# nghiapq77/face-recognition-cpp-tensorrt

Hardware: AMD Instinct MI355X
Metric: faces/sec end-to-end (detect+embed+match), 640x640 batch=32, 1M gallery (higher is better)
Workload: dtype f16 MFMA recogniser convs (fp32 accumulate) + fp32-accurate detector (fp32 MFMA, fp16 hi/lo-split MFMA for the 64-channel 3x3 convs) + int8-screened coarse scan (fp16 MFMA on exactly widened int8 rows) + exact f32 re-rank match (bit-identical to the exact f32 scan)

## Files before the change

### face-recognition-cpp-tensorrt_amd/csrc/kernels_arc_s2.hip

```cpp
#include "frt_kernels.h"
#include "frt_se_device.h"

#include <type_traits>

namespace {

constexpr int PROW = 144;

__device__ constexpr int kSub[9] = {0, 0, 0, 0, 1, 2, 2, 3, 3};
__device__ constexpr int kDr[9] = {0, 0, 1, 1, 0, 0, 1, 0, 0};
__device__ constexpr int kDc[9] = {0, 1, 0, 1, 0, 0, 0, 0, 1};
__device__ constexpr int kLen[4] = {4, 1, 2, 2};
__device__ constexpr int kRowPar[4] = {1, 0, 1, 0};
__device__ constexpr int kColPar[4] = {1, 0, 0, 1};

template <int NT, int PP, bool SEP = false, bool SCF = false>
__global__ __launch_bounds__(256, 1) void conv_s2_kernel(ConvMfmaArgs p, int R, int n_img, int linear) {
    constexpr int PLANE_B = PP * 4096;
    constexpr int LA = 2, WR = 3, BFD = 2;
    extern __shared__ __attribute__((aligned(16))) char smem[];
    const int tid = threadIdx.x, lane = tid & 63, wave = tid >> 6;
    const int r = lane & 31, hi = lane >> 5;
    const int H = p.H, W = p.W, Ho = p.Ho, Wo = p.Wo, Wq = Wo + 1;
    const int NPp = n_img * (R + 1) * Wq;
    const int strips_per_img = Ho / R;
    const int n_valid = n_img * R * Wo;

    const int n_co_tiles = p.Cout >> 7;
    const int nblk = gridDim.x, bq = nblk >> 3, brem = nblk & 7;
    const int xcd = blockIdx.x & 7, slot = blockIdx.x >> 3;
    const int lid = (xcd < brem ? xcd * (bq + 1) : brem * (bq + 1) + (xcd - brem) * bq) + slot;
    const int co_tile = lid % n_co_tiles, strip = lid / n_co_tiles;
    const int co_base = co_tile * 128, cow = wave * 32;
    const int img0 = (strip / strips_per_img) * n_img;
    const int oy0 = (strip % strips_per_img) * R;
    const int n_chunks = p.Cin >> 6;

    int poff[4][PP];
    const int n_sc = SCF ? (p.Csc >> 6) : 0;
    int poff_sc[SCF ? PP : 1];
    {
        const int plane_px = (R + 1) * Wq;
        const float inv_plane = 1.0f / (float)plane_px, inv_row = 1.0f / (float)Wq;
#pragma unroll
        for (int q = 0; q < PP; ++q) {
            const int g = (q * 4 + wave) * 64 + lane;
            const int px = g / 9, pos = g - px * 9;
            int il = (int)(((float)px + 0.5f) * inv_plane);
            int rem = px - il * plane_px;
            if (rem < 0) { --il; rem += plane_px; } else if (rem >= plane_px) { ++il; rem -= plane_px; }
            int i = (int)(((float)rem + 0.5f) * inv_row);
            int j = rem - i * Wq;
            if (j < 0) { --i; j += Wq; } else if (j >= Wq) { ++i; j -= Wq; }
            const int b = img0 + il;
            const bool live = pos < 8 && px < NPp && b < p.B;
            const int ye = 2 * (oy0 + i), xe = 2 * j;
#pragma unroll
            for (int s = 0; s < 4; ++s) {
                const int y = ye - kRowPar[s], x = xe - kColPar[s];
                poff[s][q] = (live && y >= 0 && y < H && x >= 0 && x < W) ? ((b * H + y) * W + x) * p.Cin + pos * 8 : -1;
            }
            if constexpr (SCF) poff_sc[q] = (live && ye < H && xe < W) ? ((b * H + ye) * W + xe) * p.Csc + pos * 8 : -1;
        }
    }
    const half_t *wfrag = p.wf + ((long)((co_base + cow) >> 5) * n_chunks) * (9 * 4 * 512) + lane * 8;
    int pbase[NT];
#pragma unroll
    for (int j = 0; j < NT; ++j) {
        const int sl = j * 32 + r;
        int pidx = 0;
        if (linear) {
            pidx = sl < R * Wq ? sl : 0;
        } else if (sl < n_valid) {
            const int per = R * Wo;
            int il = (int)(((float)sl + 0.5f) * (1.0f / (float)per));
            int rem = sl - il * per;
            if (rem < 0) { --il; rem += per; } else if (rem >= per) { ++il; rem -= per; }
            int rr = (int)(((float)rem + 0.5f) * (1.0f / (float)Wo));
            int cc = rem - rr * Wo;
            if (cc < 0) { --rr; cc += Wo; } else if (cc >= Wo) { ++rr; cc -= Wo; }
            pidx = (il * (R + 1) + rr) * Wq + cc;
        }
        pbase[j] = pidx * PROW + hi * 16;
    }

    half8 areg[WR][4];
    auto load_w = [&](int c, int step, auto slot_c) {
        constexpr int S = decltype(slot_c)::value;
        const int woff = c < n_chunks ? (c * 9 + step) * (4 * 512) : 0;
#pragma unroll
        for (int kk = 0; kk < 4; ++kk) areg[S][kk] = *reinterpret_cast<const half8 *>(wfrag + woff + kk * 512);
    };
    auto issue_plane = [&](int c, auto sub_c) {
        constexpr int S = decltype(sub_c)::value;
        const bool real = c < n_chunks;
        char *pl = smem + S * PLANE_B + wave * 1024;
#pragma unroll
        for (int q = 0; q < PP; ++q) {
            const half_t *src = (real && poff[S][q] >= 0) ? p.x + (unsigned)(poff[S][q] + (c << 6)) : p.zeros;
            if constexpr (SCF) {
                if (!real && S < n_sc && poff_sc[q] >= 0) src = p.scx + (unsigned)(poff_sc[q] + (S << 6));
            }
            __builtin_amdgcn_global_load_lds((const __attribute__((address_space(1))) void *)src,
                                             (__attribute__((address_space(3))) void *)(pl + q * 4096), 16, 0, 0);
        }
    };

    floatx16 acc[NT];
#pragma unroll
    for (int j = 0; j < NT; ++j)
#pragma unroll
        for (int e = 0; e < 16; ++e) acc[j][e] = 0.f;

    issue_plane(0, std::integral_constant<int, 0>{});
    issue_plane(0, std::integral_constant<int, 1>{});
    issue_plane(0, std::integral_constant<int, 2>{});
    issue_plane(0, std::integral_constant<int, 3>{});
    load_w(0, 0, std::integral_constant<int, 0>{});
    load_w(0, 1, std::integral_constant<int, 1>{});
    half8 bf[BFD][NT];
    asm volatile("s_waitcnt vmcnt(%0)" ::"n"(4 * LA) : "memory");
    __builtin_amdgcn_s_barrier();
#pragma unroll
    for (int k2 = 0; k2 < BFD; ++k2)
#pragma unroll
        for (int j = 0; j < NT; ++j) bf[k2][j] = *reinterpret_cast<const half8 *>(smem + pbase[j] + k2 * 32);

    auto step = [&](int c, auto step_c) {
        constexpr int ST = decltype(step_c)::value;
        constexpr int NS = (ST + 1) % 9;
        constexpr int AS = ST % WR;
        constexpr bool LAST_OF_PLANE = kSub[NS] != kSub[ST];
        const int dp = kSub[ST] * PLANE_B + (kDr[ST] * Wq + kDc[ST]) * PROW;
        const int dpn = kSub[NS] * PLANE_B + (kDr[NS] * Wq + kDc[NS]) * PROW;
#pragma unroll
        for (int kk = 0; kk < 4; ++kk) {
            const int cur = kk & 1;
            if (kk == 4 - BFD && LAST_OF_PLANE) {
                constexpr int NEXT = kSub[NS];
                constexpr int YOUNGER = 4 * (9 - kLen[NEXT]) + 2 * PP;
                static_assert(YOUNGER <= 63, "vmcnt field");
                asm volatile("s_waitcnt vmcnt(%0)" ::"n"(YOUNGER) : "memory");
                asm volatile("s_waitcnt lgkmcnt(0)" ::: "memory");
                __builtin_amdgcn_s_barrier();
                __builtin_amdgcn_sched_barrier(0);
                issue_plane(c + 1, std::integral_constant<int, kSub[ST]>{});
                __builtin_amdgcn_sched_barrier(0);
            }
#pragma unroll
            for (int j = 0; j < NT; ++j) {
                acc[j] = __builtin_amdgcn_mfma_f32_32x32x16_f16(areg[AS][kk], bf[cur][j], acc[j], 0, 0, 0);
                if (kk + BFD < 4) bf[cur][j] = *reinterpret_cast<const half8 *>(smem + pbase[j] + dp + (kk + BFD) * 32);
                else bf[cur][j] = *reinterpret_cast<const half8 *>(smem + pbase[j] + dpn + (kk + BFD - 4) * 32);
                if (kk == 0 && j == (NT > 1 ? 1 : 0)) {
                    constexpr int T2 = ST + LA;
                    load_w(T2 < 9 ? c : c + 1, T2 % 9, std::integral_constant<int, (T2 % 9) % WR>{});
                }
                __builtin_amdgcn_sched_barrier(0);
            }
        }
    };
    for (int c = 0; c < n_chunks; ++c) {
        step(c, std::integral_constant<int, 0>{});
        step(c, std::integral_constant<int, 1>{});
        step(c, std::integral_constant<int, 2>{});
        step(c, std::integral_constant<int, 3>{});
        step(c, std::integral_constant<int, 4>{});
        step(c, std::integral_constant<int, 5>{});
        step(c, std::integral_constant<int, 6>{});
        step(c, std::integral_constant<int, 7>{});
        step(c, std::integral_constant<int, 8>{});
    }
    floatx16 acc_sc[SCF ? NT : 1];
    if constexpr (SCF) {
        half8 wsc[4][4];
        const half_t *wsf = p.wscf + ((long)((co_base + cow) >> 5) * n_sc) * (4 * 512) + lane * 8;
#pragma unroll
        for (int c = 0; c < 4; ++c)
#pragma unroll
            for (int kk = 0; kk < 4; ++kk) wsc[c][kk] = *reinterpret_cast<const half8 *>(wsf + ((c < n_sc ? c : 0) * 4 + kk) * 512);
#pragma unroll
        for (int j = 0; j < NT; ++j)
#pragma unroll
            for (int e = 0; e < 16; ++e) acc_sc[j][e] = 0.f;
        asm volatile("s_waitcnt vmcnt(0)" ::: "memory");
        __syncthreads();
#pragma unroll
        for (int c = 0; c < 4; ++c) {
            if (c < n_sc) {
#pragma unroll
                for (int kk = 0; kk < 4; ++kk)
#pragma unroll
                    for (int j = 0; j < NT; ++j) {
                        const half8 b = *reinterpret_cast<const half8 *>(smem + pbase[j] + c * PLANE_B + kk * 32);
                        acc_sc[j] = __builtin_amdgcn_mfma_f32_32x32x16_f16(wsc[c][kk], b, acc_sc[j], 0, 0, 0);
                    }
            }
        }
    } else {
        asm volatile("s_waitcnt vmcnt(0)" ::: "memory");
    }
    __syncthreads();

    constexpr int EROW = 36;
    float *ep = reinterpret_cast<float *>(smem) + wave * (32 * EROW);
    const int chunk = lane & 3;
    const int cch = co_base + cow + chunk * 8;
    floatx4 q0[2], q1[2], q2[2], q3[2];
    q0[0] = *reinterpret_cast<const floatx4 *>(p.p0 + cch);
    q0[1] = *reinterpret_cast<const floatx4 *>(p.p0 + cch + 4);
    q1[0] = *reinterpret_cast<const floatx4 *>(p.p1 + cch);
    q1[1] = *reinterpret_cast<const floatx4 *>(p.p1 + cch + 4);
    const bool two = p.mode == EPI_BN_ADD_BN && p.out1;
    if (two) {
        q2[0] = *reinterpret_cast<const floatx4 *>(p.p2 + cch);
        q2[1] = *reinterpret_cast<const floatx4 *>(p.p2 + cch + 4);
        q3[0] = *reinterpret_cast<const floatx4 *>(p.p3 + cch);
        q3[1] = *reinterpret_cast<const floatx4 *>(p.p3 + cch + 4);
    }
    const long Mtot = (long)p.B * Ho * Wo;
    const float inv_wq = 1.0f / (float)Wq;
    auto slot_pixel = [&](int sl, long &m) -> bool {
        if (linear) {
            const int rr = (int)(((float)sl + 0.5f) * inv_wq);
            const int cc = sl - rr * Wq;
            m = ((long)img0 * Ho + oy0 + rr) * Wo + cc;
            return rr < R && cc < Wo && m < Mtot;
        }
        m = ((long)img0 * Ho + oy0) * Wo + sl;
        return sl < n_valid && m < Mtot;
    };
    if constexpr (SEP) {
        const int per_img = R * Wo;
        se_tail_epilogue<NT, (NT == 4 ? 2 : 1)>(p, acc, ep, reinterpret_cast<float *>(smem + 4 * 32 * EROW * 4), strip % strips_per_img, strips_per_img,
                                               n_co_tiles, img0, n_img, Ho * Wo, co_base, cow, [&](int sl, long &m, int &il) -> bool {
                                                   il = (NT == 4 && !linear && sl >= per_img) ? 1 : 0;
                                                   return slot_pixel(sl, m);
                                               });
        return;
    }
    half8 sc8[SCF ? 1 : NT][2];
    floatx4 qs0[2], qs1[2];
    if constexpr (SCF) {
        qs0[0] = *reinterpret_cast<const floatx4 *>(p.psc0 + cch);
        qs0[1] = *reinterpret_cast<const floatx4 *>(p.psc0 + cch + 4);
        qs1[0] = *reinterpret_cast<const floatx4 *>(p.psc1 + cch);
        qs1[1] = *reinterpret_cast<const floatx4 *>(p.psc1 + cch + 4);
    } else if (p.mode == EPI_BN_ADD_BN) {
#pragma unroll
        for (int j = 0; j < NT; ++j)
#pragma unroll
            for (int it = 0; it < 2; ++it) {
                const int sl = j * 32 + (lane >> 2) + 16 * it;
                long m;
                const bool ok = slot_pixel(sl, m);
                sc8[j][it] = *reinterpret_cast<const half8 *>(p.sc + (ok ? m : 0) * p.Cout + cch);
            }
    }
#pragma unroll
    for (int j = 0; j < NT; ++j) {
        float v[2][8];
#pragma unroll
        for (int g = 0; g < 4; ++g) {
            const floatx4 t = {acc[j][4 * g], acc[j][4 * g + 1], acc[j][4 * g + 2], acc[j][4 * g + 3]};
            *reinterpret_cast<floatx4 *>(ep + r * EROW + 8 * g + 4 * hi) = t;
        }
#pragma unroll
        for (int it = 0; it < 2; ++it) {
            const int px = (lane >> 2) + 16 * it;
            const floatx4 v0 = *reinterpret_cast<const floatx4 *>(ep + px * EROW + chunk * 8);
            const floatx4 v1 = *reinterpret_cast<const floatx4 *>(ep + px * EROW + chunk * 8 + 4);
            const float t[8] = {v0[0], v0[1], v0[2], v0[3], v1[0], v1[1], v1[2], v1[3]};
#pragma unroll
            for (int e = 0; e < 8; ++e) v[it][e] = t[e] * q0[e >> 2][e & 3] + q1[e >> 2][e & 3];
        }
        if constexpr (SCF) {
#pragma unroll
            for (int g = 0; g < 4; ++g) {
                const floatx4 t = {acc_sc[j][4 * g], acc_sc[j][4 * g + 1], acc_sc[j][4 * g + 2], acc_sc[j][4 * g + 3]};
                *reinterpret_cast<floatx4 *>(ep + r * EROW + 8 * g + 4 * hi) = t;
            }
#pragma unroll
            for (int it = 0; it < 2; ++it) {
                const int px = (lane >> 2) + 16 * it;
                const floatx4 v0 = *reinterpret_cast<const floatx4 *>(ep + px * EROW + chunk * 8);
                const floatx4 v1 = *reinterpret_cast<const floatx4 *>(ep + px * EROW + chunk * 8 + 4);
                const float t[8] = {v0[0], v0[1], v0[2], v0[3], v1[0], v1[1], v1[2], v1[3]};
#pragma unroll
                for (int e = 0; e < 8; ++e) v[it][e] += t[e] * qs0[e >> 2][e & 3] + qs1[e >> 2][e & 3];
            }
        } else if (p.mode == EPI_BN_ADD_BN) {
#pragma unroll
            for (int it = 0; it < 2; ++it)
#pragma unroll
                for (int e = 0; e < 8; ++e) v[it][e] += (float)sc8[j][it][e];
        }
#pragma unroll
        for (int it = 0; it < 2; ++it) {
            const int sl = j * 32 + (lane >> 2) + 16 * it;
            long m;
            if (!slot_pixel(sl, m)) continue;
            half8 o;
#pragma unroll
            for (int e = 0; e < 8; ++e) o[e] = (half_t)v[it][e];
            *reinterpret_cast<half8 *>(p.out0 + m * p.Cout + cch) = o;
            if (two) {
                half8 z;
#pragma unroll
                for (int e = 0; e < 8; ++e) z[e] = (half_t)(v[it][e] * q2[e >> 2][e & 3] + q3[e >> 2][e & 3]);
                *reinterpret_cast<half8 *>(p.out1 + m * p.Cout + cch) = z;
            }
        }
    }
}

constexpr int C64_ROW = 113 * 128;
constexpr int C64_LDS = 3 * C64_ROW + 2 * 32 * 36 * 4;
__global__ __launch_bounds__(128, 2) void conv_s2c64_kernel(ConvMfmaArgs p, int n_rows) {
    constexpr int Wo = 56, Ho = 56, W = 112, H = 112;
    extern __shared__ __attribute__((aligned(16))) char smem[];
    const int tid = threadIdx.x, lane = tid & 63, wave = tid >> 6;
    const int r = lane & 31, hi = lane >> 5;
    const int nblk = gridDim.x, bq = nblk >> 3, brem = nblk & 7;
    const int xcd = blockIdx.x & 7, slot = blockIdx.x >> 3;
    const int lid = (xcd < brem ? xcd * (bq + 1) : brem * (bq + 1) + (xcd - brem) * bq) + slot;
    const int row_begin = (int)((long)lid * n_rows / nblk), row_end = (int)((long)(lid + 1) * n_rows / nblk);

    constexpr int EROW = 36;
    float *ep = reinterpret_cast<float *>(smem + 3 * C64_ROW) + wave * (32 * EROW);
    const int chunk = lane & 3;
    const int cch = wave * 32 + chunk * 8;

    half8 areg[9][4];
    {
        const half_t *wfrag = p.wf + (long)wave * (9 * 4 * 512) + lane * 8;
#pragma unroll
        for (int t = 0; t < 9; ++t)
#pragma unroll
            for (int kk = 0; kk < 4; ++kk) areg[t][kk] = *reinterpret_cast<const half8 *>(wfrag + (t * 4 + kk) * 512);
    }
    auto prm = [&](int a, int t) -> float * {
        return reinterpret_cast<float *>(smem + 3 * C64_ROW) + (a >> 1) * (32 * EROW) + ((((a & 1) << 6) + t) >> 2) * EROW + 32 + (t & 3);
    };
    if (tid < 64) {
        const bool two0 = p.mode == EPI_BN_ADD_BN && p.out1;
        *prm(0, tid) = p.p0[tid];
        *prm(1, tid) = p.p1[tid];
        *prm(2, tid) = two0 ? p.p2[tid] : 0.f;
        *prm(3, tid) = two0 ? p.p3[tid] : 0.f;
    }
    if (tid < 24) {
        const int sl = tid >> 3, c = tid & 7;
        *reinterpret_cast<floatx4 *>(smem + sl * C64_ROW + c * 16) = floatx4{0.f, 0.f, 0.f, 0.f};
    }
    const int dpx = lane >> 3, dc = lane & 7;
    const int src_even = dpx * 64 + ((dc ^ (((1 + dpx) >> 1) & 7)) << 3);
    const int src_odd = dpx * 64 + ((dc ^ ((((1 + dpx) >> 1) + 4) & 7)) << 3);
    auto fetch_row = [&](const half_t *img, int y, int k0, int k1) {
        char *dst = smem + ((y + 1) % 3) * C64_ROW + 128;
        const bool row_ok = y >= 0;
        const half_t *rowp = img + y * (W * 64);
#pragma unroll
        for (int k = 0; k < 14; ++k) {
            if (k < k0 || k >= k1) continue;
            const half_t *src = row_ok ? rowp + k * 512 + ((k & 1) ? src_odd : src_even) : p.zeros;
            __builtin_amdgcn_global_load_lds((const __attribute__((address_space(1))) void *)src,
                                             (__attribute__((address_space(3))) void *)(dst + k * 1024), 16, 0, 0);
        }
    };
    auto fetch = [&](int row, bool fresh) {
        const int b = row / Ho, oy = row - b * Ho;
        const half_t *img = p.x + (long)b * (H * W * 64);
        if (fresh) fetch_row(img, 2 * oy - 1, wave * 7, wave * 7 + 7);
        fetch_row(img, 2 * oy + wave, 0, 14);
    };

    if (row_begin < row_end) fetch(row_begin, true);
    int boff[2][2];
#pragma unroll
    for (int j = 0; j < 2; ++j)
#pragma unroll
        for (int h = 0; h < 2; ++h) {
            const int sl = j * 32 + r;
            boff[j][h] = sl * 256 + ((hi ^ ((sl + h) & 7)) << 4);
        }
    asm volatile("s_waitcnt vmcnt(0)" ::: "memory");
    for (int row = row_begin; row < row_end; ++row) {
        const int b = row / Ho, oy = row - b * Ho;
        __syncthreads();

        floatx16 acc[2];
#pragma unroll
        for (int j = 0; j < 2; ++j)
#pragma unroll
            for (int e = 0; e < 16; ++e) acc[j][e] = 0.f;
#pragma unroll
        for (int kh = 0; kh < 3; ++kh) {
            const char *rowb = smem + ((2 * oy + kh) % 3) * C64_ROW;
#pragma unroll
            for (int kw = 0; kw < 3; ++kw)
#pragma unroll
                for (int kk = 0; kk < 4; ++kk)
#pragma unroll
                    for (int j = 0; j < 2; ++j) {
                        const half8 bf = *reinterpret_cast<const half8 *>(rowb + ((boff[j][kw >> 1] ^ (kk << 5)) + kw * 128));
                        acc[j] = __builtin_amdgcn_mfma_f32_32x32x16_f16(areg[kh * 3 + kw][kk], bf, acc[j], 0, 0, 0);
                    }
        }
        __syncthreads();
        if (row + 1 < row_end) fetch(row + 1, oy + 1 == Ho);

        const bool two = p.mode == EPI_BN_ADD_BN && p.out1;
        const long m0 = ((long)b * Ho + oy) * Wo;
        const long s0 = p.mode == EPI_BN_ADD_BN ? ((long)b * p.sc_h + oy * p.sc_stride) * p.sc_w : 0;
#pragma unroll
        for (int j = 0; j < 2; ++j) {
            asm volatile("" ::: "memory");
            half8 sc8[2];
#pragma unroll
            for (int it = 0; it < 2; ++it) {
                const int sl = j * 32 + (lane >> 2) + 16 * it;
                if (p.mode == EPI_BN_ADD_BN) sc8[it] = *reinterpret_cast<const half8 *>(p.sc + (s0 + (sl < Wo ? sl * p.sc_stride : 0)) * 64 + cch);
            }
            floatx4 q0[2], q1[2], q2[2], q3[2];
#pragma unroll
            for (int h = 0; h < 2; ++h) {
                q0[h] = *reinterpret_cast<const floatx4 *>(prm(0, cch + 4 * h));
                q1[h] = *reinterpret_cast<const floatx4 *>(prm(1, cch + 4 * h));
                q2[h] = *reinterpret_cast<const floatx4 *>(prm(2, cch + 4 * h));
                q3[h] = *reinterpret_cast<const floatx4 *>(prm(3, cch + 4 * h));
            }
#pragma unroll
            for (int g = 0; g < 4; ++g) {
                const floatx4 v = {acc[j][4 * g], acc[j][4 * g + 1], acc[j][4 * g + 2], acc[j][4 * g + 3]};
                *reinterpret_cast<floatx4 *>(ep + r * EROW + 8 * g + 4 * hi) = v;
            }
#pragma unroll
            for (int it = 0; it < 2; ++it) {
                const int px = (lane >> 2) + 16 * it;
                const floatx4 v0 = *reinterpret_cast<const floatx4 *>(ep + px * EROW + chunk * 8);
                const floatx4 v1 = *reinterpret_cast<const floatx4 *>(ep + px * EROW + chunk * 8 + 4);
                const int sl = j * 32 + px;
                if (sl >= Wo) continue;
                float v[8] = {v0[0], v0[1], v0[2], v0[3], v1[0], v1[1], v1[2], v1[3]};
#pragma unroll
                for (int e = 0; e < 8; ++e) v[e] = v[e] * q0[e >> 2][e & 3] + q1[e >> 2][e & 3];
                if (p.mode == EPI_BN_ADD_BN) {
#pragma unroll
                    for (int e = 0; e < 8; ++e) v[e] += (float)sc8[it][e];
                }
                half8 o;
#pragma unroll
                for (int e = 0; e < 8; ++e) o[e] = (half_t)v[e];
                *reinterpret_cast<half8 *>(p.out0 + (m0 + sl) * 64 + cch) = o;
                if (two) {
                    half8 z;
#pragma unroll
                    for (int e = 0; e < 8; ++e) z[e] = (half_t)(v[e] * q2[e >> 2][e & 3] + q3[e >> 2][e & 3]);
                    *reinterpret_cast<half8 *>(p.out1 + (m0 + sl) * 64 + cch) = z;
                }
            }
        }
        if (two) asm volatile("s_waitcnt vmcnt(8)" ::: "memory");
        else asm volatile("s_waitcnt vmcnt(4)" ::: "memory");
    }
}

bool s2c64_applies(const ConvMfmaArgs &a) {
    if (!a.wf2 || a.ks != 3 || a.stride != 2 || a.pad != 1 || a.Cout != 64 || a.Cin != 64 || a.splits != 1 || (a.H & 1) || (a.W & 1)) return false;
    if (a.Ho * 2 != a.H || a.Wo * 2 != a.W || a.Wo != 56 || a.Ho != 56) return false;
    if (a.mode != EPI_BN && a.mode != EPI_BN_ADD_BN) return false;
    return a.mode != EPI_BN_ADD_BN || a.sc;
}

template <int NT, int PP, bool SEP = false, bool SCF = false>
void launch_s2_t(const ConvMfmaArgs &a0, const ConvPlan &p, hipStream_t s) {
    constexpr size_t lds = (size_t)4 * PP * 4096;
    static_assert(lds <= 160 * 1024 && lds >= 4 * 32 * 36 * 4, "LDS budget / epilogue scratch");
    static bool attr_done[FRT_MAX_DEVICES] = {};
    if (frt_first_use_on_device(attr_done))
        (void)hipFuncSetAttribute(reinterpret_cast<const void *>(&conv_s2_kernel<NT, PP, SEP, SCF>), hipFuncAttributeMaxDynamicSharedMemorySize, (int)lds);
    ConvMfmaArgs a = a0;
    a.wf = a0.wf2;
    const int strips = ((a.B + p.n_img - 1) / p.n_img) * (a.Ho / p.R);
    const int linear = (p.n_img == 1 && p.R * (a.Wo + 1) <= NT * 32) ? 1 : 0;
    hipLaunchKernelGGL((conv_s2_kernel<NT, PP, SEP, SCF>), dim3(strips * (a.Cout / 128)), dim3(256), lds, s, a, p.R, p.n_img, linear);
}

void launch_s2c64(const ConvMfmaArgs &a0, const ConvPlan &, hipStream_t s) {
    ConvMfmaArgs a = a0;
    a.wf = a0.wf2;
    static bool attr_done[FRT_MAX_DEVICES] = {};
    if (frt_first_use_on_device(attr_done))
        (void)hipFuncSetAttribute(reinterpret_cast<const void *>(&conv_s2c64_kernel), hipFuncAttributeMaxDynamicSharedMemorySize, C64_LDS);
    const int n_rows = a.B * a.Ho;
    hipLaunchKernelGGL(conv_s2c64_kernel, dim3(n_rows < 768 ? n_rows : 768), dim3(128), C64_LDS, s, a, n_rows);
}

bool s2_geometry(const ConvMfmaArgs &a, int &R, int &n_img, int &nt, int &pp) {
    if (!a.wf2 || a.ks != 3 || a.stride != 2 || a.pad != 1 || a.Cout % 128 || a.Cin % 64 || a.splits != 1 || a.H != a.W || (a.H & 1)) return false;
    if (a.Ho * 2 != a.H || a.Wo * 2 != a.W) return false;
    if (a.mode != EPI_BN && a.mode != EPI_BN_ADD_BN && a.mode != EPI_BN_SE) return false;
    const bool scf = a.mode == EPI_BN_ADD_BN && a.scx;
    if (scf && !(a.wscf && a.psc0 && a.psc1 && (a.Csc == 64 || a.Csc == 128 || a.Csc == 256))) return false;
    if (!scf && (a.mode == EPI_BN_ADD_BN || a.mode == EPI_BN_SE) && !(a.sc && a.sc_stride == 1 && a.sc_h == a.Ho && a.sc_w == a.Wo)) return false;
    const int Wq = a.Wo + 1;
    if (a.Ho * a.Wo <= 64) {
        R = a.Ho;
        n_img = (a.B >= 96 && 2 * a.Ho * a.Wo <= 128) ? 2 : 1;
        nt = n_img * a.Ho * a.Wo <= 64 ? 2 : 4;
    } else {
        n_img = 1;
        R = 0;
        for (int d = a.Ho; d >= 1; --d) {
            if (a.Ho % d || d * Wq > 224) continue;
            R = d;
            break;
        }
        if (!R) return false;
        nt = R * Wq <= 128 ? 4 : 7;
        if (R * a.Wo * 10 < nt * 32 * 7) return false;
    }
    pp = (n_img * (R + 1) * Wq * 9 + 255) / 256;
    return pp <= 9;
}

enum { S2_C64, S2_7, S2_7_SCF, S2_7_SE, S2_4, S2_4_SCF, S2_4_SE, S2_4W, S2_4W_SCF, S2_2, S2_2_SCF };
const ConvRow kS2[] = {
     {"conv_s2c64_kernel", launch_s2c64, -1},
     {"conv_s2_kernel<7, 9, false, false>", launch_s2_t<7, 9>, S2_7_SE},
     {"conv_s2_kernel<7, 9, false, true>", launch_s2_t<7, 9, false, true>, -1},
     {"conv_s2_kernel<7, 9, true, false>", launch_s2_t<7, 9, true>, -1},
     {"conv_s2_kernel<4, 5, false, false>", launch_s2_t<4, 5>, S2_4_SE},
     {"conv_s2_kernel<4, 5, false, true>", launch_s2_t<4, 5, false, true>, -1},
     {"conv_s2_kernel<4, 5, true, false>", launch_s2_t<4, 5, true>, -1},
     {"conv_s2_kernel<4, 9, false, false>", launch_s2_t<4, 9>, -1},
     {"conv_s2_kernel<4, 9, false, true>", launch_s2_t<4, 9, false, true>, -1},
     {"conv_s2_kernel<2, 5, false, false>", launch_s2_t<2, 5>, -1},
     {"conv_s2_kernel<2, 5, false, true>", launch_s2_t<2, 5, false, true>, -1},
};

}

bool plan_s2(const ConvMfmaArgs &a, ConvPlan &p) {
    if (s2c64_applies(a)) {
        conv_plan_row(p, CONV_S2, kS2, S2_C64);
        return true;
    }
    int R, n_img, nt, pp;
    if (!s2_geometry(a, R, n_img, nt, pp)) return false;
    const bool scf = a.mode == EPI_BN_ADD_BN && a.scx;
    const int base = nt == 7 ? S2_7 : (nt == 4 ? (pp <= 5 ? S2_4 : S2_4W) : S2_2);
    conv_plan_row(p, CONV_S2, kS2, base + (scf ? 1 : 0));
    p.R = R;
    p.n_img = n_img;
    p.uses_scx = scf;
    const bool se_geom = nt == 7 ? (n_img == 1 && a.Ho / R <= SE_SPLIT) : (n_img == 2 ? R == a.Ho : (n_img == 1 && a.Ho / R <= SE_SPLIT));
    if (se_geom) conv_plan_se_twin(p, kS2, a);
    return true;
}

void launch_s2(const ConvMfmaArgs &a, const ConvPlan &p, hipStream_t s) { kS2[p.row].launch(a, p, s); }
```

Measured before the change: 45110.

## Hand-schedule vmcnt waits and issue weight/LDS-DMA loads via inline asm in s2 conv

Replaces the compiler-generated weight fragment loads and global_load_lds calls with inline asm that uses wave-uniform scalar bases and immediate offsets. Adds a constexpr model of the vmcnt ordering so each step waits only for the loads it needs, and double-buffers the shortcut-conv B fragment reads from LDS. The aim is to drop compiler-inserted conservative waits and address arithmetic so MFMA overlaps better with the loads. In exchange, correctness now rests on hand-counted vmcnt values and asm register constraints, which is fragile.

```diff
diff --git a/face-recognition-cpp-tensorrt_amd/csrc/frt_arc_vmsched.hpp b/face-recognition-cpp-tensorrt_amd/csrc/frt_arc_vmsched.hpp
--- /dev/null
+++ b/face-recognition-cpp-tensorrt_amd/csrc/frt_arc_vmsched.hpp
@@ -0,0 +1,56 @@
+#pragma once
+
+namespace frt_vmsched {
+
+constexpr int kFrag = 4;
+
+constexpr int kS2Plane[9] = {0, 0, 0, 0, 1, 2, 2, 3, 3};
+constexpr int kS2Len[4] = {4, 1, 2, 2};
+
+constexpr bool s2_hands_over(int step) { return kS2Plane[(step + 1) % 9] != kS2Plane[step]; }
+
+constexpr int s2_step_wait(int PP, int LA, int step) {
+    int n = kFrag * (LA - 1);
+    for (int d = 1; d <= LA; ++d)
+        if (s2_hands_over(((step - d) % 9 + 9) % 9)) n += PP;
+    return n;
+}
+
+constexpr int s2_handover_wait(int PP, int next) { return kFrag * (9 - kS2Len[next]) + 2 * PP; }
+
+struct S2Counts {
+    int step[9];
+    int handover[4];
+};
+constexpr S2Counts s2_counts(int PP, int LA) {
+    S2Counts c{};
+    for (int t = 0; t < 9; ++t) c.step[t] = s2_step_wait(PP, LA, t);
+    for (int s = 0; s < 4; ++s) c.handover[s] = s2_handover_wait(PP, s);
+    return c;
+}
+
+template <class Sink>
+void s2_replay(int PP, int LA, int n_chunks, const S2Counts &cnt, Sink &&sink) {
+    for (int s = 0; s < 4; ++s)
+        for (int q = 0; q < PP; ++q) sink.dma(0, s);
+    for (int t = 0; t < LA; ++t)
+        for (int k = 0; k < kFrag; ++k) sink.frag(0, t);
+    sink.wait(0, true);
+    sink.read(0, 0);
+    for (int c = 0; c < n_chunks; ++c)
+        for (int t = 0; t < 9; ++t) {
+            sink.wait(cnt.step[t], false);
+            sink.mfma(c, t);
+            const int t2 = t + LA;
+            for (int k = 0; k < kFrag; ++k) sink.frag(c + t2 / 9, t2 % 9);
+            if (s2_hands_over(t)) {
+                const int next = kS2Plane[(t + 1) % 9];
+                sink.wait(cnt.handover[next], true);
+                sink.read(t == 8 ? c + 1 : c, next);
+                for (int q = 0; q < PP; ++q) sink.dma(c + 1, kS2Plane[t]);
+            }
+        }
+    sink.wait(0, true);
+}
+
+}
diff --git a/face-recognition-cpp-tensorrt_amd/csrc/kernels_arc_s2.hip b/face-recognition-cpp-tensorrt_amd/csrc/kernels_arc_s2.hip
--- a/face-recognition-cpp-tensorrt_amd/csrc/kernels_arc_s2.hip
+++ b/face-recognition-cpp-tensorrt_amd/csrc/kernels_arc_s2.hip
@@ -1,9 +1,20 @@
+#include "frt_arc_vmsched.hpp"
 #include "frt_kernels.h"
 #include "frt_se_device.h"
 
 #include <type_traits>
+#include <utility>
 
 namespace {
+
+template <class F, int... I>
+__device__ __forceinline__ void static_for_impl(F &&f, std::integer_sequence<int, I...>) {
+    (f(std::integral_constant<int, I>{}), ...);
+}
+template <int N, class F>
+__device__ __forceinline__ void static_for(F &&f) {
+    static_for_impl(f, std::make_integer_sequence<int, N>{});
+}
 
 constexpr int PROW = 144;
 
@@ -13,6 +24,12 @@
 __device__ constexpr int kLen[4] = {4, 1, 2, 2};
 __device__ constexpr int kRowPar[4] = {1, 0, 1, 0};
 __device__ constexpr int kColPar[4] = {1, 0, 0, 1};
+static_assert(kSub[0] == frt_vmsched::kS2Plane[0] && kSub[1] == frt_vmsched::kS2Plane[1] && kSub[2] == frt_vmsched::kS2Plane[2] &&
+                  kSub[3] == frt_vmsched::kS2Plane[3] && kSub[4] == frt_vmsched::kS2Plane[4] && kSub[5] == frt_vmsched::kS2Plane[5] &&
+                  kSub[6] == frt_vmsched::kS2Plane[6] && kSub[7] == frt_vmsched::kS2Plane[7] && kSub[8] == frt_vmsched::kS2Plane[8],
+              "step -> plane");
+static_assert(kLen[0] == frt_vmsched::kS2Len[0] && kLen[1] == frt_vmsched::kS2Len[1] && kLen[2] == frt_vmsched::kS2Len[2] && kLen[3] == frt_vmsched::kS2Len[3],
+              "steps per plane");
 
 template <int NT, int PP, bool SEP = false, bool SCF = false>
 __global__ __launch_bounds__(256, 1) void conv_s2_kernel(ConvMfmaArgs p, int R, int n_img, int linear) {
@@ -21,6 +38,7 @@
     extern __shared__ __attribute__((aligned(16))) char smem[];
     const int tid = threadIdx.x, lane = tid & 63, wave = tid >> 6;
     const int r = lane & 31, hi = lane >> 5;
+    const int wave_u = __builtin_amdgcn_readfirstlane(wave);
     const int H = p.H, W = p.W, Ho = p.Ho, Wo = p.Wo, Wq = Wo + 1;
     const int NPp = n_img * (R + 1) * Wq;
     const int strips_per_img = Ho / R;
@@ -63,7 +81,9 @@
             if constexpr (SCF) poff_sc[q] = (live && ye < H && xe < W) ? ((b * H + ye) * W + xe) * p.Csc + pos * 8 : -1;
         }
     }
-    const half_t *wfrag = p.wf + ((long)((co_base + cow) >> 5) * n_chunks) * (9 * 4 * 512) + lane * 8;
+    const half_t *wfrag = p.wf + ((long)((co_base + wave_u * 32) >> 5) * n_chunks) * (9 * 4 * 512);
+    const unsigned lane_off = lane * 16;
+    const unsigned plane_lds = (unsigned)(size_t)(__attribute__((address_space(3))) char *)smem + wave_u * 1024;
     int pbase[NT];
 #pragma unroll
     for (int j = 0; j < NT; ++j) {
@@ -88,22 +108,30 @@
     auto load_w = [&](int c, int step, auto slot_c) {
         constexpr int S = decltype(slot_c)::value;
         const int woff = c < n_chunks ? (c * 9 + step) * (4 * 512) : 0;
-#pragma unroll
-        for (int kk = 0; kk < 4; ++kk) areg[S][kk] = *reinterpret_cast<const half8 *>(wfrag + woff + kk * 512);
+        half8(&d)[4] = areg[S];
+        const half_t *src = wfrag + woff;
+        const unsigned lo = lane_off;
+        asm volatile("s_nop 4\n\t"
+                     "global_load_dwordx4 %0, %4, %5\n\t"
+                     "global_load_dwordx4 %1, %4, %5 offset:1024\n\t"
+                     "global_load_dwordx4 %2, %4, %5 offset:2048\n\t"
+                     "global_load_dwordx4 %3, %4, %5 offset:3072"
+                     : "=&v"(d[0]), "=&v"(d[1]), "=&v"(d[2]), "=&v"(d[3])
+                     : "v"(lo), "s"(src)
+                     : "memory");
     };
     auto issue_plane = [&](int c, auto sub_c) {
         constexpr int S = decltype(sub_c)::value;
         const bool real = c < n_chunks;
-        char *pl = smem + S * PLANE_B + wave * 1024;
-#pragma unroll
-        for (int q = 0; q < PP; ++q) {
+        static_for<PP>([&](auto q_c) {
+            constexpr int q = decltype(q_c)::value;
             const half_t *src = (real && poff[S][q] >= 0) ? p.x + (unsigned)(poff[S][q] + (c << 6)) : p.zeros;
             if constexpr (SCF) {
                 if (!real && S < n_sc && poff_sc[q] >= 0) src = p.scx + (unsigned)(poff_sc[q] + (S << 6));
             }
-            __builtin_amdgcn_global_load_lds((const __attribute__((address_space(1))) void *)src,
-                                             (__attribute__((address_space(3))) void *)(pl + q * 4096), 16, 0, 0);
-        }
+            const unsigned base = plane_lds;
+            asm volatile("s_add_u32 m0, %0, %1\n\ts_nop 0\n\tglobal_load_lds_dwordx4 %2, off" ::"s"(base), "n"(S * PLANE_B + q * 4096), "v"(src) : "memory", "scc");
+        });
     };
 
     floatx16 acc[NT];
@@ -119,8 +147,10 @@
     load_w(0, 0, std::integral_constant<int, 0>{});
     load_w(0, 1, std::integral_constant<int, 1>{});
     half8 bf[BFD][NT];
-    asm volatile("s_waitcnt vmcnt(%0)" ::"n"(4 * LA) : "memory");
+    asm volatile("s_waitcnt vmcnt(0)" ::: "memory");
+    __builtin_amdgcn_s_waitcnt(0xc07f);
     __builtin_amdgcn_s_barrier();
+    __builtin_amdgcn_sched_barrier(0);
 #pragma unroll
     for (int k2 = 0; k2 < BFD; ++k2)
 #pragma unroll
@@ -133,12 +163,14 @@
         constexpr bool LAST_OF_PLANE = kSub[NS] != kSub[ST];
         const int dp = kSub[ST] * PLANE_B + (kDr[ST] * Wq + kDc[ST]) * PROW;
         const int dpn = kSub[NS] * PLANE_B + (kDr[NS] * Wq + kDc[NS]) * PROW;
+        asm volatile("s_waitcnt vmcnt(%0)" ::"n"(frt_vmsched::s2_step_wait(PP, LA, ST)) : "memory");
+        __builtin_amdgcn_sched_barrier(0);
 #pragma unroll
         for (int kk = 0; kk < 4; ++kk) {
             const int cur = kk & 1;
             if (kk == 4 - BFD && LAST_OF_PLANE) {
                 constexpr int NEXT = kSub[NS];
-                constexpr int YOUNGER = 4 * (9 - kLen[NEXT]) + 2 * PP;
+                constexpr int YOUNGER = frt_vmsched::s2_handover_wait(PP, NEXT);
                 static_assert(YOUNGER <= 63, "vmcnt field");
                 asm volatile("s_waitcnt vmcnt(%0)" ::"n"(YOUNGER) : "memory");
                 asm volatile("s_waitcnt lgkmcnt(0)" ::: "memory");
@@ -171,6 +203,14 @@
         step(c, std::integral_constant<int, 7>{});
         step(c, std::integral_constant<int, 8>{});
     }
+    auto wait_all = [&]() {
+        asm volatile("s_waitcnt vmcnt(0)"
+                     : "+v"(areg[0][0]), "+v"(areg[0][1]), "+v"(areg[0][2]), "+v"(areg[0][3]), "+v"(areg[1][0]), "+v"(areg[1][1]), "+v"(areg[1][2]),
+                       "+v"(areg[1][3]), "+v"(areg[2][0]), "+v"(areg[2][1]), "+v"(areg[2][2]), "+v"(areg[2][3])
+                     :
+                     : "memory");
+    };
+    static_assert(WR == 3, "wait_all names the ring's registers");
     floatx16 acc_sc[SCF ? NT : 1];
     if constexpr (SCF) {
         half8 wsc[4][4];
@@ -183,8 +223,13 @@
         for (int j = 0; j < NT; ++j)
 #pragma unroll
             for (int e = 0; e < 16; ++e) acc_sc[j][e] = 0.f;
-        asm volatile("s_waitcnt vmcnt(0)" ::: "memory");
+        wait_all();
         __syncthreads();
+        half8 bs[BFD][NT];
+#pragma unroll
+        for (int k2 = 0; k2 < BFD; ++k2)
+#pragma unroll
+            for (int j = 0; j < NT; ++j) bs[k2][j] = *reinterpret_cast<const half8 *>(smem + pbase[j] + k2 * 32);
 #pragma unroll
         for (int c = 0; c < 4; ++c) {
             if (c < n_sc) {
@@ -192,13 +237,15 @@
                 for (int kk = 0; kk < 4; ++kk)
 #pragma unroll
                     for (int j = 0; j < NT; ++j) {
-                        const half8 b = *reinterpret_cast<const half8 *>(smem + pbase[j] + c * PLANE_B + kk * 32);
-                        acc_sc[j] = __builtin_amdgcn_mfma_f32_32x32x16_f16(wsc[c][kk], b, acc_sc[j], 0, 0, 0);
+                        constexpr int cur_mask = BFD - 1;
+                        const int cur = kk & cur_mask, nx = c * 4 + kk + BFD;
+                        acc_sc[j] = __builtin_amdgcn_mfma_f32_32x32x16_f16(wsc[c][kk], bs[cur][j], acc_sc[j], 0, 0, 0);
+                        if (nx < 16) bs[cur][j] = *reinterpret_cast<const half8 *>(smem + pbase[j] + (nx >> 2) * PLANE_B + (nx & 3) * 32);
                     }
             }
         }
     } else {
-        asm volatile("s_waitcnt vmcnt(0)" ::: "memory");
+        wait_all();
     }
     __syncthreads();
 
```

Measured after the change: 45500 (median of 6 runs). No clear change (+0.9%).
